# philip-bl/dctn

Measured on AMD Instinct MI355X. Metric: EPS-contraction windows/sec (fwd+bwd), higher is better.
Workload: dtype bf16; 1 GPU; cfg2 EPS[(3,4)]+linear bf16 B1024/GPU; parallelism=dp1

## Files before the change

dctn_amd/csrc/eps_mfma.hip:

```cpp
#include "common.h"

#include <cstdlib>
#include <type_traits>

typedef __attribute__((ext_vector_type(8))) __bf16 bf16x8;
typedef __attribute__((ext_vector_type(16))) float f32x16;
typedef __attribute__((ext_vector_type(8))) float f32x8;
typedef __attribute__((ext_vector_type(2))) int int2v;
typedef __attribute__((ext_vector_type(4))) int int4v;
typedef __attribute__((ext_vector_type(2))) float f32x2;

namespace {

constexpr int ilog2(int v) { return v <= 1 ? 0 : 1 + ilog2(v >> 1); }

template <typename S> __device__ __forceinline__ float to_f32(S v) { return (float)v; }

__device__ __forceinline__ float half_sum(float v) {
  const int iv = __float_as_int(v);
  const int2v r = __builtin_amdgcn_permlane32_swap(iv, iv, false, false);
  return __int_as_float(r[0]) + __int_as_float(r[1]);
}

__device__ __forceinline__ void swap_halves(float& a, float& b) {
// ... 38 lines not shown
  return t;
}
__device__ __forceinline__ bf16x8 tr_frag(const short* tile, int ks, const TrLane& t) {
  typedef __attribute__((address_space(3))) s16x4 lds_s16x4;
  const s16x4 lo = __builtin_amdgcn_ds_read_tr16_b64_v4i16((lds_s16x4*)(tile + t.rd_lo + ks * 16 * LROW));
  const s16x4 hi = __builtin_amdgcn_ds_read_tr16_b64_v4i16((lds_s16x4*)(tile + t.rd_hi + ks * 16 * LROW));
  const s16x8 v = {lo[0], lo[1], lo[2], lo[3], hi[0], hi[1], hi[2], hi[3]};
  return __builtin_bit_cast(bf16x8, v);
}

struct FastDiv {
  unsigned M, s1, s2;
};
__device__ __forceinline__ unsigned fdiv(unsigned n, const FastDiv& d) {
  const unsigned t = __umulhi(d.M, n);
  return (t + ((n - t) >> d.s1)) >> d.s2;
}

#define MFMA_MAXN 16
struct MfmaP {
  int C, B, K, O, Ho, Wo;
  int P;
  int npg;
  int spc, nchunks;
  unsigned foffb[MFMA_MAXN];
  unsigned rowoffb[MFMA_MAXN];
  unsigned s1b, s2b, s3b, s4b;
  unsigned x_bytes;
  unsigned o_bytes, o_s1b;
  FastDiv div_wo;
  int rowvec_ok;
  int vec_ok;
  int Cout;
  unsigned hw_rowb, hw_bytes;
  int ncb;
  int skew;
  int opts;
#ifdef DCTN_STAMPS
  unsigned long long* stamps;
#endif
};

#ifdef DCTN_STAMPS
#define DCTN_STAMP(P, SLOT)                                                                      \
  do {                                                                                           \
    __builtin_amdgcn_sched_barrier(0);                                                           \
    unsigned long long t_;                                                                       \
    asm volatile("s_memrealtime %0\n\ts_waitcnt lgkmcnt(0)" : "=s"(t_)::"memory");               \
    if ((P).stamps && threadIdx.x == 0) (P).stamps[(long long)blockIdx.x * 8 + (SLOT)] = t_;     \
    __builtin_amdgcn_sched_barrier(0);                                                           \
  } while (0)
static unsigned long long* g_stamps = nullptr;
void dctn_stamps_set(unsigned long long* p) { g_stamps = p; }
__device__ unsigned long long* g_dev_stamps = nullptr;
void dctn_reduce_stamps_set(unsigned long long* p) { (void)hipMemcpyToSymbol(HIP_SYMBOL(g_dev_stamps), &p, sizeof(p)); }
#define DCTN_STAMP_T(P, SLOT, TID)                                                              \
  do {                                                                                           \
    __builtin_amdgcn_sched_barrier(0);                                                           \
    unsigned long long t_;                                                                       \
    asm volatile("s_memrealtime %0\n\ts_waitcnt lgkmcnt(0)" : "=s"(t_)::"memory");               \
    if ((P).stamps && threadIdx.x == (TID)) (P).stamps[(long long)blockIdx.x * 8 + (SLOT)] = t_;  \
    __builtin_amdgcn_sched_barrier(0);                                                           \
  } while (0)
#define DCTN_STAMP_ROLE_ROW 1024
#define DCTN_STAMP_R(P, SLOT)                                                                    \
  do {                                                                                           \
    __builtin_amdgcn_sched_barrier(0);                                                           \
    unsigned long long t_;                                                                       \
    asm volatile("s_memrealtime %0\n\ts_waitcnt lgkmcnt(0)" : "=s"(t_)::"memory");               \
    if ((P).stamps && threadIdx.x == 64 * 8)                                                     \
      (P).stamps[(long long)(DCTN_STAMP_ROLE_ROW + blockIdx.x) * 8 + (SLOT)] = t_;               \
    __builtin_amdgcn_sched_barrier(0);                                                           \
  } while (0)
#define DCTN_STAMP_WAVE_ROW 1536
#define DCTN_STAMP_W(P, WV)                                                                      \
  do {                                                                                           \
    __builtin_amdgcn_sched_barrier(0);                                                           \
    unsigned long long t_;                                                                       \
    asm volatile("s_memrealtime %0\n\ts_waitcnt lgkmcnt(0)" : "=s"(t_)::"memory");               \
    if ((P).stamps && (threadIdx.x & 63) == 0 && (WV) < 8)                                        \
      (P).stamps[(long long)(DCTN_STAMP_WAVE_ROW + blockIdx.x) * 8 + (WV)] = t_;                 \
    __builtin_amdgcn_sched_barrier(0);                                                           \
  } while (0)
#define DCTN_STAMP_G(SLOT)                                                                       \
  do {                                                                                           \
    __builtin_amdgcn_sched_barrier(0);                                                           \
    unsigned long long t_;                                                                       \
    asm volatile("s_memrealtime %0\n\ts_waitcnt lgkmcnt(0)" : "=s"(t_)::"memory");               \
    if (g_dev_stamps && threadIdx.x == 0) g_dev_stamps[(long long)blockIdx.x * 8 + (SLOT)] = t_;  \
    __builtin_amdgcn_sched_barrier(0);                                                           \
  } while (0)
#else
#define DCTN_STAMP(P, SLOT) do { } while (0)
#define DCTN_STAMP_T(P, SLOT, TID) do { } while (0)
#define DCTN_STAMP_G(SLOT) do { } while (0)
#define DCTN_STAMP_R(P, SLOT) do { } while (0)
#define DCTN_STAMP_W(P, WV) do { } while (0)
#endif

typedef __attribute__((ext_vector_type(4))) unsigned u32x4;
typedef __attribute__((ext_vector_type(2))) unsigned u32x2;
typedef __attribute__((ext_vector_type(2))) __bf16 bf16x2;

__device__ __forceinline__ __amdgpu_buffer_rsrc_t make_rsrc(const void* ptr, unsigned bytes) {
  return __builtin_amdgcn_make_buffer_rsrc(const_cast<void*>(ptr), 0, (int)bytes, 0x00020000);
}

template <typename S, int N, bool VEC, int ROWS>
struct RawWindow {
  u32x4 row[ROWS > 0 ? ROWS : 1];
  unsigned v[(ROWS == 0 && VEC) ? N * (int)(sizeof(S) / 2) : 1];
  unsigned e[(ROWS == 0 && !VEC) ? 2 * N : 1];
};

template <typename S, int N, bool VEC, int ROWS>
__device__ __forceinline__ void issue_window(__amdgpu_buffer_rsrc_t rs, unsigned voff, unsigned soff,
                                             const MfmaP& p, RawWindow<S, N, VEC, ROWS>& raw) {
  if constexpr (ROWS > 0) {
#pragma unroll
    for (int rw = 0; rw < ROWS; ++rw)
      raw.row[rw] = __builtin_amdgcn_raw_buffer_load_b128(rs, voff, soff + p.rowoffb[rw], 0);
  } else if constexpr (VEC) {
#pragma unroll
    for (int n = 0; n < N; ++n) {
      if constexpr (sizeof(S) == 2) {
        raw.v[n] = __builtin_amdgcn_raw_buffer_load_b32(rs, voff, soff + p.foffb[n], 0);
      } else {
        const u32x2 t = __builtin_amdgcn_raw_buffer_load_b64(rs, voff, soff + p.foffb[n], 0);
        raw.v[2 * n] = t.x;
        raw.v[2 * n + 1] = t.y;
      }
    }
  } else {
#pragma unroll
    for (int n = 0; n < N; ++n)
#pragma unroll
      for (int q = 0; q < 2; ++q) {
        if constexpr (sizeof(S) == 2)
          raw.e[2 * n + q] = (unsigned)(unsigned short)__builtin_amdgcn_raw_buffer_load_b16(
              rs, voff, soff + p.foffb[n] + q * p.s4b, 0);
        else
          raw.e[2 * n + q] = __builtin_amdgcn_raw_buffer_load_b32(rs, voff, soff + p.foffb[n] + q * p.s4b, 0);
      }
  }
}

template <typename S, int N, bool VEC, int ROWS>
__device__ __forceinline__ void unpack_window(const RawWindow<S, N, VEC, ROWS>& raw, float (&xv)[N][2]) {
  if constexpr (ROWS > 0) {
    constexpr int KK = N / ROWS;
    constexpr int CC = ROWS * ROWS / N;
#pragma unroll
    for (int rw = 0; rw < ROWS; ++rw) {
      const unsigned d[4] = {raw.row[rw].x, raw.row[rw].y, raw.row[rw].z, raw.row[rw].w};
#pragma unroll
      for (int dw = 0; dw < KK; ++dw) {
        const int n = ((rw / CC) * KK + dw) * CC + (rw % CC);
        xv[n][0] = __uint_as_float(d[dw] << 16);
        xv[n][1] = __uint_as_float(d[dw] & 0xffff0000u);
      }
    }
  } else if constexpr (VEC) {
#pragma unroll
    for (int n = 0; n < N; ++n) {
      if constexpr (sizeof(S) == 2) {
        xv[n][0] = __uint_as_float(raw.v[n] << 16);
        xv[n][1] = __uint_as_float(raw.v[n] & 0xffff0000u);
      } else {
        xv[n][0] = __uint_as_float(raw.v[2 * n]);
        xv[n][1] = __uint_as_float(raw.v[2 * n + 1]);
      }
    }
  } else {
#pragma unroll
    for (int n = 0; n < N; ++n)
#pragma unroll
      for (int q = 0; q < 2; ++q)
        xv[n][q] = sizeof(S) == 2 ? __uint_as_float(raw.e[2 * n + q] << 16) : __uint_as_float(raw.e[2 * n + q]);
  }
}
// ... 403 lines not shown
        for (int bh = 0; bh < BN / 2; ++bh) {
          const f32x2 mm = bmul2(ph[bh], f32x2{xv[N - 1][0], xv[N - 1][1]});
          m0[bh] = mm[0];
          m1[bh] = mm[1];
          swap_halves(m0[bh], m1[bh]);
        }
      }
      float res0[OP], res1[OP];
#pragma unroll
      for (int o = 0; o < OP; ++o) { res0[o] = 0.f; res1[o] = 0.f; }
#pragma unroll
      for (int t = 0; t < MT; ++t) {
#pragma unroll
        for (int set = 0; set < 2; ++set) {
          f32x16 acc;
#pragma unroll
          for (int v = 0; v < 16; ++v) acc[v] = 0.f;
#pragma unroll
          for (int s = 0; s < KS; ++s)
            acc = __builtin_amdgcn_mfma_f32_32x32x16_bf16(cf[t][s], set ? pf1[s] : pf0[s], acc, 0, 0, 0);
#pragma unroll
          for (int v = 0; v < 16; v += 2) {
            const int code = (t << 4) | ((v >> 2) << 2) | (v & 3);
            const float mm = set ? m1[code >> LOGO] : m0[code >> LOGO];
            float* dst = set ? res1 : res0;
            const int o = code & (OP - 1);
            const f32x2 r = bfma2(mm, f32x2{acc[v], acc[v + 1]}, f32x2{dst[o], dst[o + 1]});
            dst[o] = r[0];
            dst[o + 1] = r[1];
          }
        }
      }
      unsigned pk[OP / 2];
#pragma unroll
      for (int i = 0; i < OP / 2; ++i) {
        float a0 = res0[2 * i], a1 = res1[2 * i], c0 = res0[2 * i + 1], c1 = res1[2 * i + 1];
        swap_halves(a0, a1);
        swap_halves(c0, c1);
        pk[i] = pack_bf16(a0 + a1, c0 + c1);
      }
      if constexpr (OP == 2) {
        __builtin_amdgcn_raw_buffer_store_b32(pk[0], rs_o, voff_o, (unsigned)b * p.o_s1b, 0);
        *reinterpret_cast<unsigned*>(tile + (b - g0) * SROW + lane * OP) = pk[0];
      } else if constexpr (OP == 4) {
        __builtin_amdgcn_raw_buffer_store_b64(u32x2{pk[0], pk[1]}, rs_o, voff_o, (unsigned)b * p.o_s1b, 0);
        *reinterpret_cast<u32x2*>(tile + (b - g0) * SROW + lane * OP) = u32x2{pk[0], pk[1]};
      } else {
#pragma unroll
        for (int i = 0; i < OP / 8; ++i) {
          const u32x4 q = u32x4{pk[4 * i], pk[4 * i + 1], pk[4 * i + 2], pk[4 * i + 3]};
          __builtin_amdgcn_raw_buffer_store_b128(q, rs_o, voff_o, (unsigned)b * p.o_s1b + 16u * i, 0);
          *reinterpret_cast<u32x4*>(tile + (b - g0) * SROW + lane * OP + 8 * i) = q;
        }
      }
      if (b == b0) DCTN_STAMP(p, 2);
    }
    wave_lds_sync();
    f32x4v hd = {0.f, 0.f, 0.f, 0.f};
#pragma unroll
    for (int ks = 0; ks < HK; ++ks) {
      const bf16x8 fb = *reinterpret_cast<const bf16x8*>(brd + 32 * ks);
      hd = __builtin_amdgcn_mfma_f32_16x16x32_bf16(wf[ks], fb, hd, 0, 0, 0);
    }
    wave_lds_sync();
    {
      const int sl = lane & 15, cb = 4 * (lane >> 4);
      if (sl < g1 - g0) {
#pragma unroll
        for (int v = 0; v < 4; ++v) hsum[grp & 1][sl][cb + v][wv] = hd[v];
      }
    }
    DCTN_STAMP(p, 3);
    __syncthreads();
    for (int e = tid; e < (g1 - g0) * p.Cout; e += (int)blockDim.x) {
      const int sl = e / p.Cout, c = e - sl * p.Cout;
      float t = (float)bias[c];
      for (int w = 0; w < nwv; ++w) t += hsum[grp & 1][sl][c][w];
      logits[(long long)(g0 + sl) * p.Cout + c] = (bf16_t)t;
    }
  }
  DCTN_STAMP(p, 4);
}

constexpr int HEADT_WAVES = 16;
constexpr int HEADT_GS = 4;
constexpr int HEADT_MAXKS = 6;
constexpr int headt_pitch(int F) { return (F + 31) / 32 * 32 + 8; }

template <int N0, int N1, int OP, int ROWS, bool BLK4>
__global__ __launch_bounds__(64 * HEADT_WAVES) void eps_fwd_head_q2reg_t_k(const bf16_t* __restrict__ x,
                                                                           const bf16_t* __restrict__ core,
                                                                           const bf16_t* __restrict__ hw,
                                                                           const bf16_t* __restrict__ bias,
                                                                           bf16_t* __restrict__ out,
                                                                           bf16_t* __restrict__ logits, MfmaP p) {
  typedef bf16_t S;
  typedef __attribute__((ext_vector_type(4))) float f32x4v;
  constexpr int N = N0 + N1, A = 1 << N0, BN = 1 << N1, KS = A / 16, MT = BN * OP / 32;
  constexpr int LOGO = ilog2(OP);
  constexpr int TOT = A * BN * OP;
  static_assert(OP % 2 == 0 && TOT % 4 == 0, "outputs are handled as bf16 pairs");
  __shared__ __attribute__((aligned(16))) bf16_t cs[TOT];
  __shared__ float hsum[HEADT_WAVES][HEADT_GS][16];
  __shared__ unsigned step_ctr;
  extern __shared__ __attribute__((aligned(16))) short ftile[];
  const int tid = threadIdx.x, lane = tid & 63;
  const int wv = __builtin_amdgcn_readfirstlane(tid >> 6);
  const int b0 = (int)blockIdx.x * p.spc, b1 = b0 + p.spc < p.B ? b0 + p.spc : p.B;
  const int F = p.P * OP, LP = headt_pitch(F);
  const __amdgpu_buffer_rsrc_t rs_x = make_rsrc(x, p.x_bytes), rs_o = make_rsrc(out, p.o_bytes);
  __shared__ float bias_s[16];
  DCTN_STAMP(p, 0);
  float bias_v = 0.f;
  for (int e0 = 0; e0 < TOT; e0 += 4 * 64 * HEADT_WAVES) {
    S tmp[4];
#pragma unroll
    for (int i = 0; i < 4; ++i) {
      const int ec = e0 + tid + i * 64 * HEADT_WAVES, e = ec < TOT ? ec : TOT - 1, o = e % OP, ab = e / OP;
      tmp[i] = core[(long long)ab * p.O + (o < p.O ? o : 0)];
    }
    if (e0 == 0 && wv == 0) bias_v = (float)bias[(lane & 15) < p.Cout ? (lane & 15) : 0];
#pragma unroll
    for (int i = 0; i < 4; ++i) {
      const int e = e0 + tid + i * 64 * HEADT_WAVES, o = e % OP, ab = e / OP, bb = ab % BN, aa = ab / BN;
      const int code = ((bb >> 1) << LOGO) | o;
      const int row = (((code >> 2) & 3) << 3) | ((bb & 1) << 2) | (code & 3);
      const int dst = ((((code >> 4) * KS + (aa >> 4)) * 64 + ((aa >> 3) & 1) * 32 + row) << 3) | (aa & 7);
      if (e < TOT) cs[dst] = o < p.O ? tmp[i] : (bf16_t)0.f;
    }
  }
  if (wv == 0) bias_s[lane & 15] = bias_v;
  for (int e = tid; e < HEADT_GS * (LP - F); e += 64 * HEADT_WAVES) ftile[(e / (LP - F)) * LP + F + e % (LP - F)] = 0;
  __syncthreads();
  bf16x8 cf[MT][KS];
#pragma unroll
  for (int t = 0; t < MT; ++t)
#pragma unroll
    for (int s = 0; s < KS; ++s)
      cf[t][s] = *reinterpret_cast<const bf16x8*>(&cs[((t * KS + s) * 64 + lane) * 8]);
  DCTN_STAMP(p, 1);

  auto lane_at = [&](int pg, bool live, unsigned& voff_x, unsigned& voff_o, int& pos) {
    pos = pg * 64 + lane;
    const bool valid = live && pos < p.P;
    const unsigned pu = (unsigned)(pos < p.P ? pos : p.P - 1);
    const unsigned ho = fdiv(pu, p.div_wo), wo = pu - ho * (unsigned)p.Wo;
    voff_x = valid ? ho * p.s2b + wo * p.s3b : p.x_bytes;
    voff_o = valid ? pu * (unsigned)(OP * 2) : p.o_bytes;
  };
  auto draw = [&]() {
    unsigned v = 0;
    if (lane == 0) v = __hip_atomic_fetch_add(&step_ctr, 1u, __ATOMIC_RELAXED, __HIP_MEMORY_SCOPE_WORKGROUP);
    return (int)__builtin_amdgcn_readfirstlane(v);
  };

  for (int g0 = b0; g0 < b1; g0 += HEADT_GS) {
    const int ng = g0 + HEADT_GS < b1 ? HEADT_GS : b1 - g0;
    const int nsteps = ng * p.npg;
    if (tid == 0) step_ctr = 2 * HEADT_WAVES;
    __syncthreads();
    int cur = wv, nxt = wv + HEADT_WAVES;
    int s = cur / p.npg, pg = cur - s * p.npg, pos;
    unsigned voff_x, voff_o;
    lane_at(pg, cur < nsteps, voff_x, voff_o, pos);
    RawWindow<S, N, true, ROWS> raw;
    issue_window<S, N, true, ROWS>(rs_x, voff_x, (unsigned)(g0 + (cur < nsteps ? s : 0)) * p.s1b, p, raw);
#ifdef DCTN_STAMPS
    bool first_step = true;
#endif
    while (cur < nsteps) {
      float xv[N][2];
      unpack_window<S, N, true, ROWS>(raw, xv);
      const unsigned vo = voff_o, so = (unsigned)(g0 + s) * p.o_s1b;
      short* trow = ftile + s * LP + (pos < p.P ? pos : 0) * OP;
      const bool tvalid = pos < p.P;
      {
        cur = nxt;
        s = cur / p.npg;
        pg = cur - s * p.npg;
        lane_at(pg, cur < nsteps, voff_x, voff_o, pos);
        issue_window<S, N, true, ROWS>(rs_x, voff_x, (unsigned)(g0 + (cur < nsteps ? s : 0)) * p.s1b, p, raw);
        nxt = draw();
        __builtin_amdgcn_sched_barrier(0);
      }
      bf16x8 pf0[KS], pf1[KS];
      build_p0<N0>(xv, pf0, pf1);
#pragma unroll
      for (int s2 = 0; s2 < KS; ++s2) swap_halves(pf0[s2], pf1[s2]);
      float m0[BN / 2], m1[BN / 2];
      {
        float ph[BN / 2];
        ph[0] = xv[N - 2][0];
        ph[1] = xv[N - 2][1];
#pragma unroll
        for (int u = 2; u < N1; ++u)
#pragma unroll
          for (int bh = (1 << (u - 1)) - 1; bh >= 0; --bh) {
            const f32x2 pr = bmul2(ph[bh], f32x2{xv[N - 1 - u][0], xv[N - 1 - u][1]});
            ph[bh] = pr[0];
            ph[bh | (1 << (u - 1))] = pr[1];
          }
#pragma unroll
        for (int bh = 0; bh < BN / 2; ++bh) {
          const f32x2 mm = bmul2(ph[bh], f32x2{xv[N - 1][0], xv[N - 1][1]});
          m0[bh] = mm[0];
          m1[bh] = mm[1];
          swap_halves(m0[bh], m1[bh]);
        }
      }
      float res0[OP], res1[OP];
#pragma unroll
      for (int o = 0; o < OP; ++o) { res0[o] = 0.f; res1[o] = 0.f; }
#pragma unroll
      for (int t = 0; t < MT; ++t) {
#pragma unroll
        for (int set = 0; set < 2; ++set) {
          f32x16 acc;
#pragma unroll
          for (int v = 0; v < 16; ++v) acc[v] = 0.f;
#pragma unroll
          for (int s2 = 0; s2 < KS; ++s2)
            acc = __builtin_amdgcn_mfma_f32_32x32x16_bf16(cf[t][s2], set ? pf1[s2] : pf0[s2], acc, 0, 0, 0);
#pragma unroll
          for (int v = 0; v < 16; v += 2) {
            const int code = (t << 4) | ((v >> 2) << 2) | (v & 3);
            const float mm = set ? m1[code >> LOGO] : m0[code >> LOGO];
            float* dst = set ? res1 : res0;
            const int o = code & (OP - 1);
            const f32x2 r = __builtin_elementwise_fma(f32x2{mm, mm}, f32x2{acc[v], acc[v + 1]}, f32x2{dst[o], dst[o + 1]});
            dst[o] = r[0];
            dst[o + 1] = r[1];
          }
        }
      }
      unsigned pk[OP / 2];
#pragma unroll
      for (int i = 0; i < OP / 2; ++i) {
        float a0 = res0[2 * i], a1 = res1[2 * i], c0 = res0[2 * i + 1], c1 = res1[2 * i + 1];
        swap_halves(a0, a1);
        swap_halves(c0, c1);
        pk[i] = pack_bf16(a0 + a1, c0 + c1);
      }
      if constexpr (OP == 2) {
        if constexpr (!BLK4) __builtin_amdgcn_raw_buffer_store_b32(pk[0], rs_o, vo, so, 0);
        if (tvalid) *reinterpret_cast<unsigned*>(trow) = pk[0];
      } else if constexpr (OP == 4) {
        if constexpr (!BLK4) __builtin_amdgcn_raw_buffer_store_b64(u32x2{pk[0], pk[1]}, rs_o, vo, so, 0);
        if (tvalid) *reinterpret_cast<u32x2*>(trow) = u32x2{pk[0], pk[1]};
      } else {
#pragma unroll
        for (int i = 0; i < OP / 8; ++i) {
          const u32x4 q = u32x4{pk[4 * i], pk[4 * i + 1], pk[4 * i + 2], pk[4 * i + 3]};
          if constexpr (!BLK4) __builtin_amdgcn_raw_buffer_store_b128(q, rs_o, vo, so + 16u * i, 0);
          if (tvalid) *reinterpret_cast<u32x4*>(trow + 8 * i) = q;
        }
      }
#ifdef DCTN_STAMPS
      if (first_step) DCTN_STAMP(p, 2);
      first_step = false;
#endif
    }
    DCTN_STAMP(p, 3);
    DCTN_STAMP_T(p, 4, 64 * (HEADT_WAVES - 1));
    const int nks = (F + 31) / 32;
    const int c = lane & 15, kg = lane >> 4;
    const __amdgpu_buffer_rsrc_t rs_hw = make_rsrc(hw, p.hw_bytes);
    u32x4 wf[HEADT_MAXKS];
#pragma unroll
    for (int i = 0; i < HEADT_MAXKS; ++i) {
      const int ks = wv + HEADT_WAVES * i, k = 32 * ks + 8 * kg;
      const unsigned vo2 = (ks < nks && c < p.Cout && k + 7 < F) ? (unsigned)c * p.hw_rowb + (unsigned)k * 2u : p.hw_bytes;
      wf[i] = __builtin_amdgcn_raw_buffer_load_b128(rs_hw, vo2, 0, 0);
    }
    __syncthreads();
    DCTN_STAMP(p, 5);
    if constexpr (BLK4) {
      static_assert(HEADT_GS == 4, "a group is one block of the blocked4 layout");
      const unsigned sob = (unsigned)(g0 >> 2) * (unsigned)F * 8u;
      for (int f = 2 * tid; f < F; f += 2 * 64 * HEADT_WAVES) {
        unsigned r[HEADT_GS];
#pragma unroll
        for (int i = 0; i < HEADT_GS; ++i) r[i] = i < ng ? *reinterpret_cast<const unsigned*>(ftile + i * LP + f) : 0u;
        const u32x4 q = u32x4{__builtin_amdgcn_perm(r[1], r[0], 0x05040100u), __builtin_amdgcn_perm(r[3], r[2], 0x05040100u),
                              __builtin_amdgcn_perm(r[1], r[0], 0x07060302u), __builtin_amdgcn_perm(r[3], r[2], 0x07060302u)};
        __builtin_amdgcn_raw_buffer_store_b128(q, rs_o, (unsigned)f * 8u, sob, 0);
      }
    }
    __builtin_amdgcn_sched_barrier(0);
    f32x4v hd = {0.f, 0.f, 0.f, 0.f};
    const short* brd = ftile + (c < HEADT_GS ? c : HEADT_GS - 1) * LP + 8 * kg;
#pragma unroll
    for (int i = 0; i < HEADT_MAXKS; ++i) {
      const int ks = wv + HEADT_WAVES * i;
      if (ks < nks) {
        const bf16x8 fb = *reinterpret_cast<const bf16x8*>(brd + 32 * ks);
        hd = __builtin_amdgcn_mfma_f32_16x16x32_bf16(__builtin_bit_cast(bf16x8, wf[i]), fb, hd, 0, 0, 0);
      }
    }
    if (c < HEADT_GS) {
#pragma unroll
      for (int v = 0; v < 4; ++v) hsum[wv][c][4 * kg + v] = hd[v];
    }
    __syncthreads();
    if (tid < HEADT_GS * 16) {
      const int sl = tid >> 4, cc = tid & 15;
      if (sl < ng && cc < p.Cout) {
        float t = bias_s[cc];
#pragma unroll
        for (int w = 0; w < HEADT_WAVES; ++w) t += hsum[w][sl][cc];
        logits[(long long)(g0 + sl) * p.Cout + cc] = (bf16_t)t;
      }
    }
  }
  DCTN_STAMP(p, 6);
}

constexpr int BWD_WAVES = 8;
constexpr size_t dcore_dyn_lds_bytes(int mt) { return (size_t)BWD_WAVES * (1 + mt) * 64 * 32 * sizeof(short); }

__device__ __forceinline__ void head_dw_role_waves(const bf16_t* __restrict__ feat, const bf16_t* __restrict__ dL,
                                                   bf16_t* __restrict__ dW, int B, int Cout, long long F, int n_dw,
                                                   int rw, float* __restrict__ lds, const MfmaP& p);
template <typename S, int N0, int N1, int OP, bool XVEC, bool OVEC, int ROWS, int HEADC, int DWROLE = 0>
__global__ __launch_bounds__(64 * (BWD_WAVES + DWROLE)) void eps_bwd_dcore_q2reg_k(const S* __restrict__ x,
                                                             const S* __restrict__ dY,
                                                             const S* __restrict__ hw,
                                                             const S* __restrict__ feat,
                                                             float* __restrict__ partial,
                                                             float* __restrict__ dwpart, MfmaP p,
                                                             S* __restrict__ dW, int n_dw) {
  constexpr int N = N0 + N1, A = 1 << N0, BN = 1 << N1, KS = A / 16, MT = BN * OP / 32;
  constexpr int AT = A >= 32 ? A / 32 : 1;
  constexpr int LOGO = ilog2(OP);
  constexpr bool LDST = A == 32 && MT <= 2;
  __shared__ float red[BWD_WAVES][32 * 32];
  extern __shared__ __attribute__((aligned(16))) unsigned char dsm[];
  const int tid = threadIdx.x, lane = tid & 63, r = lane & 31, h = lane >> 5, wv = tid >> 6;
  DCTN_STAMP(p, 0);
  if constexpr (DWROLE > 0) {
    static_assert(HEADC > 0 && HEADC <= 16 && LDST && OVEC && XVEC && sizeof(S) == 2 && OP == 4, "the dW role rides the HEADMM path");
    const int rw = __builtin_amdgcn_readfirstlane(wv) - BWD_WAVES;
    if (rw >= 0) {
      head_dw_role_waves(feat, dY, dW, p.B, p.Cout, (long long)p.P * OP, n_dw, rw,
                         reinterpret_cast<float*>(dsm + dcore_dyn_lds_bytes(MT) + 8192), p);
      return;
    }
#ifdef DCTN_DWROLE_PRIO
    __builtin_amdgcn_s_setprio(DCTN_DWROLE_PRIO);
#endif
  }
  short* tiles = reinterpret_cast<short*>(dsm) + wv * ((1 + MT) * 64 * LROW);
  const TrLane trl = tr_lane(lane);

  bf16x8 ident[2];
#pragma unroll
  for (int sp = 0; sp < 2; ++sp)
#pragma unroll
    for (int j = 0; j < 8; ++j) ident[sp][j] = (bf16_t)((16 * sp + 8 * h + j == r) ? 1.f : 0.f);

  f32x16 acc[MT][AT];
#pragma unroll
  for (int t = 0; t < MT; ++t)
#pragma unroll
    for (int a = 0; a < AT; ++a)
#pragma unroll
      for (int v = 0; v < 16; ++v) acc[t][a][v] = 0.f;

  const WaveJob job = wave_job(p, BWD_WAVES, (int)sizeof(S), HEADC > 0);
  const __amdgpu_buffer_rsrc_t rs_x = make_rsrc(x, p.x_bytes);
  const __amdgpu_buffer_rsrc_t rs_dy = make_rsrc(HEADC > 0 ? feat : dY, p.o_bytes);
  constexpr bool HEADMM = HEADC > 0 && HEADC <= 16 && LDST && OVEC && XVEC && sizeof(S) == 2 && OP == 4;
  float hwf[HEADC > 0 && !HEADMM ? HEADC : 1][OP];
  float dwacc[HEADC > 0 && !HEADMM ? HEADC : 1][OP];
#pragma unroll
  for (int c = 0; c < (HEADC > 0 && !HEADMM ? HEADC : 1); ++c)
#pragma unroll
    for (int o = 0; o < OP; ++o) dwacc[c][o] = 0.f;
  constexpr int DLW = HEADC > 0 ? HEADC / 2 : 1;
  const unsigned* dl32 = reinterpret_cast<const unsigned*>(dY);
  unsigned dlraw[DLW];
  RawRow<S, OP> rr[HEADC > 0 && !HEADMM ? HEADC : 1];
  constexpr bool LATE = HEADC > 0 && LDST && !HEADMM;
  auto issue_head_weight = [&]() {
    if constexpr (HEADC > 0 && !HEADMM) {
// ... 933 lines not shown
  constexpr int MT = BN * OP / 32;
  const bool headmm = A == 32 && MT <= 2 && OP == 4 && m.vec_ok;
  if (headmm && (long long)m.B * m.P * OP * 2 >= (1LL << 31)) return DCTN_ERR_UNSUPPORTED;
  const bool gemm = headmm;
  m.skew = headmm ? DCTN_DCORE_SKEW(m.spc) : 0;
  if (m.skew >= m.spc) m.skew = m.spc - 1;

  const dim3 g(grid), b(64 * BWD_WAVES);
  constexpr int NN = N0 + N1;
  constexpr int RW = NN == 9 ? 3 : 4;
  const int n_slices = (int)(((long long)m.P * OP + DWG_BFW - 1) / DWG_BFW);
  bool dwrole = false;
  if constexpr (A == 32 && MT <= 2 && OP == 4) {
    constexpr size_t RDYN = DYN + 8192 + DWR_LDS_BYTES;
#define DCTN_HEAD_ROLE_LAUNCH(ROWSV, HC)                                                                          \
  do {                                                                                                            \
    const void* kfn = (const void*)eps_bwd_dcore_q2reg_k<S, N0, N1, OP, true, true, ROWSV, HC, DWR_WAVES>;        \
    if (dctn_lds_optin(kfn, RDYN)) {                                                                              \
      hipLaunchKernelGGL((eps_bwd_dcore_q2reg_k<S, N0, N1, OP, true, true, ROWSV, HC, DWR_WAVES>), g,             \
                         dim3(64 * (BWD_WAVES + DWR_WAVES)), RDYN, st, (const S*)x, (const S*)dL, (const S*)hw,   \
                         (const S*)feat, (float*)ws, dwpart, m, (S*)dW, dW ? n_slices : 0);                       \
      dwrole = true;                                                                                              \
    }                                                                                                             \
  } while (0)
    if (blk && headmm) {
      if (m.rowvec_ok) {
        if (m.Cout <= 10) DCTN_HEAD_ROLE_LAUNCH(RW, 10); else DCTN_HEAD_ROLE_LAUNCH(RW, 16);
      } else {
        if (m.Cout <= 10) DCTN_HEAD_ROLE_LAUNCH(0, 10); else DCTN_HEAD_ROLE_LAUNCH(0, 16);
      }
    }
#undef DCTN_HEAD_ROLE_LAUNCH
  }
#define DCTN_HEAD_LAUNCH(XV, ROWSV, HC)                                                                        \
  DCTN_DCORE_LAUNCH((eps_bwd_dcore_q2reg_k<S, N0, N1, OP, XV, true, ROWSV, HC>), g, b, (DYN > 0 ? DYN + 8192 : 0), st, (const S*)x, \
                     (const S*)dL, (const S*)hw, (const S*)feat, (float*)ws, dwpart, m, (S*)nullptr, 0)
  if (dwrole) {
  } else if (m.rowvec_ok && m.vec_ok) {
    if (m.Cout <= 10) DCTN_HEAD_LAUNCH(true, RW, 10); else DCTN_HEAD_LAUNCH(true, RW, 16);
  } else if (m.vec_ok) {
    if (m.Cout <= 10) DCTN_HEAD_LAUNCH(true, 0, 10); else DCTN_HEAD_LAUNCH(true, 0, 16);
  } else {
    if (m.Cout <= 10) DCTN_HEAD_LAUNCH(false, 0, 10); else DCTN_HEAD_LAUNCH(false, 0, 16);
  }
#undef DCTN_HEAD_LAUNCH
  DCTN_CHECK_LAUNCH();
  if (m.opts & DCTN_OPT_MAIN_KERNEL_ONLY) return DCTN_PARTIAL;
  const int fw = blk ? DWG_BFW : DWG_FW;
  const int n_core = BN * OP * AT;
  if (dwrole) {
    hipLaunchKernelGGL(eps_head_reduce_k, dim3(n_core + 1), dim3(1024), 0, st, (const float*)ws, (S*)dCore, grid, A, BN, m.O, OP,
                       AT * 32, n_core, (const float*)dwpart, (S*)nullptr, m.ncb, nW, 0, (const S*)dL, (S*)dBias, m.B, m.Cout,
                       (const S*)feat, 0);
    DCTN_CHECK_LAUNCH();
    dctn_set_last_kernel("eps_head_bwd_mfma_q2reg");
    return DCTN_OK;
  }
  const int n_dw = gemm ? (int)(((long long)m.P * OP + fw - 1) / fw) : (int)((nW + 255) / 256);
  const size_t gemm_lds = (size_t)DWG_WAVES * (fw / 4) * 64 * sizeof(float);
  static_assert(DWG_WAVES * 64 == 1024, "the gemm role is the whole workgroup of eps_head_reduce_k");
  if (gemm && !dctn_lds_optin((const void*)eps_head_reduce_k, gemm_lds)) return DCTN_ERR_LAUNCH;
  hipLaunchKernelGGL(eps_head_reduce_k, dim3(n_core + n_dw + 1), dim3(1024), gemm ? gemm_lds : 0, st, (const float*)ws, (S*)dCore,
                     grid, A, BN, m.O, OP, AT * 32, n_core, (const float*)dwpart, (S*)dW, m.ncb, nW, n_dw,
                     (const S*)dL, (S*)dBias, m.B, m.Cout, (const S*)feat, gemm ? (blk ? 2 : 1) : 0);
  DCTN_CHECK_LAUNCH();
  dctn_set_last_kernel("eps_head_bwd_mfma_q2reg");
  return DCTN_OK;
}

template <int N0, int N1, int OP>
int fwd_head_launch_t(const void* x, const void* core, const void* hw, const void* bias, void* out, void* logits,
                      const MfmaP& m_in, hipStream_t st) {
  typedef bf16_t S;
  MfmaP m = m_in;
  const bool blk = (m.opts & DCTN_OPT_HEAD_FEATURES_BLOCKED4) != 0;
  if (m.O != OP || !(m.rowvec_ok && m.vec_ok) || m.npg > HEAD_FWD_MAXPG) return DCTN_ERR_UNSUPPORTED;
  if (((uintptr_t)hw % 16) != 0 || m.hw_rowb % 16 != 0 || ((uintptr_t)out % (blk ? 16 : OP * 2)) != 0) return DCTN_ERR_UNSUPPORTED;
  int nwg = m.B < dctn_dev().cus ? m.B : dctn_dev().cus;
  m.spc = (m.B + nwg - 1) / nwg;
  if (blk) m.spc = (m.spc + HEADT_GS - 1) / HEADT_GS * HEADT_GS;
  nwg = (m.B + m.spc - 1) / m.spc;
  constexpr int RW = (N0 + N1) == 9 ? 3 : 4;
  const long long F = (long long)m.P * OP;
  const bool tk = !(m.opts & DCTN_OPT_SMALL_CHUNKS) && F % 8 == 0 && F <= (long long)HEADT_WAVES * HEADT_MAXKS * 32;
  if (blk) {
    if (!tk || !head_blocked4_ok<N0, N1, OP>(m)) return DCTN_ERR_UNSUPPORTED;
    m.o_bytes = blocked4_bytes(m);
  }
  if (tk) {
    const size_t dyn = (size_t)HEADT_GS * headt_pitch((int)F) * sizeof(short);
#define DCTN_HEADT_LAUNCH(BLK)                                                                                          \
    if (!dctn_lds_optin((const void*)eps_fwd_head_q2reg_t_k<N0, N1, OP, RW, BLK>, dyn)) return DCTN_ERR_UNSUPPORTED;    \
    hipLaunchKernelGGL((eps_fwd_head_q2reg_t_k<N0, N1, OP, RW, BLK>), dim3((unsigned)nwg), dim3(64 * HEADT_WAVES), dyn, st, \
                       (const S*)x, (const S*)core, (const S*)hw, (const S*)bias, (S*)out, (S*)logits, m)
    if (blk) { DCTN_HEADT_LAUNCH(true); } else { DCTN_HEADT_LAUNCH(false); }
#undef DCTN_HEADT_LAUNCH
    DCTN_CHECK_LAUNCH();
    dctn_set_last_kernel("eps_head_fwd_mfma_q2reg");
    return DCTN_OK;
  }
  const dim3 g((unsigned)nwg), b((unsigned)(64 * m.npg));
  hipLaunchKernelGGL((eps_fwd_head_q2reg_k<N0, N1, OP, RW>), g, b, 0, st, (const S*)x, (const S*)core, (const S*)hw,
                     (const S*)bias, (S*)out, (S*)logits, m);
  DCTN_CHECK_LAUNCH();
  dctn_set_last_kernel("eps_head_fwd_mfma_q2reg");
  return DCTN_OK;
}

#define DISPATCH_OP(FN, S, N0, N1, OPV, ...)                         \
  switch (OPV) {                                                     \
    case 2: return FN<S, N0, N1, 2>(__VA_ARGS__);                    \
    case 4: return FN<S, N0, N1, 4>(__VA_ARGS__);                    \
    case 8: return FN<S, N0, N1, 8>(__VA_ARGS__);                    \
    case 16: return FN<S, N0, N1, 16>(__VA_ARGS__);                  \
  }                                                                  \
  return DCTN_ERR_UNSUPPORTED;

template <typename S>
int fwd_dispatch(const void* x, const void* core, void* out, double* stats, const MfmaP& m, int N, int op,
                 hipStream_t st) {
  if (N == 9) { DISPATCH_OP(fwd_launch_t, S, 5, 4, op, x, core, out, stats, m, st) }
  DISPATCH_OP(fwd_launch_t, S, 4, 4, op, x, core, out, stats, m, st)
}

template <typename S>
int bwd_dispatch(const void* x, const void* dY, void* dCore, void* ws, const MfmaP& m, int N,
                 int op, hipStream_t st) {
  if (N == 9) { DISPATCH_OP(bwd_launch_t, S, 5, 4, op, x, dY, dCore, ws, m, st) }
  DISPATCH_OP(bwd_launch_t, S, 4, 4, op, x, dY, dCore, ws, m, st)
}

}

int eps_fwd_mfma(const void* x, const void* core, void* out, const EpsP& p, int dtype,
                 int precision, hipStream_t st, double* stats) {
  if (!family_ok(p, dtype, precision)) return DCTN_ERR_UNSUPPORTED;
  if (!out && !stats) return DCTN_ERR_NULL;
  MfmaP m;
  fill_mp(m, p, x, dtype);
  const int op = next_pow2(p.O) < 2 ? 2 : next_pow2(p.O);
  if (dtype == DCTN_BF16) return fwd_dispatch<bf16_t>(x, core, out, stats, m, p.N, op, st);
  return fwd_dispatch<float>(x, core, out, stats, m, p.N, op, st);
}

size_t eps_bwd_mfma_workspace(const EpsP& p, int dtype, int precision, int need_dx,
                              int need_dcore) {
  (void)need_dx;
  if (!need_dcore || !family_ok(p, dtype, precision)) return 0;
  const int op = next_pow2(p.O) < 2 ? 2 : next_pow2(p.O);
  const int n0 = (p.N + 1) / 2, n1 = p.N - n0;
  const long long A = 1LL << n0, BN = 1LL << n1, acols = A >= 32 ? A : 32;
  return (size_t)dctn_dev().cus * (size_t)(BN * op) * (size_t)acols * sizeof(float);
}

int eps_bwd_mfma(const void* x, const void* core, const void* dY, void* dX, void* dCore, void* ws,
                 size_t ws_bytes, const EpsP& p, int dtype, int precision, hipStream_t st) {
  (void)core;
  if (dX || !dCore) return DCTN_ERR_UNSUPPORTED;
  if (!family_ok(p, dtype, precision)) return DCTN_ERR_UNSUPPORTED;
  if (!ws || ws_bytes < eps_bwd_mfma_workspace(p, dtype, precision, 0, 1)) return DCTN_ERR_WORKSPACE;
  MfmaP m;
  fill_mp(m, p, x, dtype);
  const int op = next_pow2(p.O) < 2 ? 2 : next_pow2(p.O);
  if (dtype == DCTN_BF16) return bwd_dispatch<bf16_t>(x, dY, dCore, ws, m, p.N, op, st);
  return bwd_dispatch<float>(x, dY, dCore, ws, m, p.N, op, st);
}

// ... 56 lines not shown
```

Measured before the change: 28.39 billion windows/s.

## Overlap forward head tail with EPS steps via per-position-group completion counters

```diff
diff --git a/dctn_amd/csrc/eps_mfma.hip b/dctn_amd/csrc/eps_mfma.hip
--- a/dctn_amd/csrc/eps_mfma.hip
+++ b/dctn_amd/csrc/eps_mfma.hip
@@ -144,6 +144,16 @@
       (P).stamps[(long long)(DCTN_STAMP_WAVE_ROW + blockIdx.x) * 8 + (WV)] = t_;                 \
     __builtin_amdgcn_sched_barrier(0);                                                           \
   } while (0)
+#define DCTN_STAMP_FWAVE_ROW 2048
+#define DCTN_STAMP_FW(P, KIND, WV)                                                               \
+  do {                                                                                           \
+    __builtin_amdgcn_sched_barrier(0);                                                           \
+    unsigned long long t_;                                                                       \
+    asm volatile("s_memrealtime %0\n\ts_waitcnt lgkmcnt(0)" : "=s"(t_)::"memory");               \
+    if ((P).stamps && (threadIdx.x & 63) == 0 && blockIdx.x < 256)                               \
+      (P).stamps[(long long)(DCTN_STAMP_FWAVE_ROW + blockIdx.x * 8 + (KIND) * 2 + ((WV) >> 3)) * 8 + ((WV) & 7)] = t_; \
+    __builtin_amdgcn_sched_barrier(0);                                                           \
+  } while (0)
 #define DCTN_STAMP_G(SLOT)                                                                       \
   do {                                                                                           \
     __builtin_amdgcn_sched_barrier(0);                                                           \
@@ -158,6 +168,7 @@
 #define DCTN_STAMP_G(SLOT) do { } while (0)
 #define DCTN_STAMP_R(P, SLOT) do { } while (0)
 #define DCTN_STAMP_W(P, WV) do { } while (0)
+#define DCTN_STAMP_FW(P, KIND, WV) do { } while (0)
 #endif
 
 typedef __attribute__((ext_vector_type(4))) unsigned u32x4;
@@ -727,6 +738,12 @@
   DCTN_STAMP(p, 4);
 }
 
+#ifdef DCTN_FWD_HEAD_SERIAL_TAIL
+constexpr bool HEADT_OVERLAP = false;
+#else
+constexpr bool HEADT_OVERLAP = true;
+#endif
+constexpr int HEADT_MAXPG = 16;
 constexpr int HEADT_WAVES = 16;
 constexpr int HEADT_GS = 4;
 constexpr int HEADT_MAXKS = 6;
@@ -748,6 +765,8 @@
   __shared__ __attribute__((aligned(16))) bf16_t cs[TOT];
   __shared__ float hsum[HEADT_WAVES][HEADT_GS][16];
   __shared__ unsigned step_ctr;
+  __shared__ unsigned tail_ctr;
+  __shared__ unsigned done[HEADT_MAXPG];
   extern __shared__ __attribute__((aligned(16))) short ftile[];
   const int tid = threadIdx.x, lane = tid & 63;
   const int wv = __builtin_amdgcn_readfirstlane(tid >> 6);
@@ -798,14 +817,41 @@
     if (lane == 0) v = __hip_atomic_fetch_add(&step_ctr, 1u, __ATOMIC_RELAXED, __HIP_MEMORY_SCOPE_WORKGROUP);
     return (int)__builtin_amdgcn_readfirstlane(v);
   };
+  auto draw_tail = [&]() {
+    unsigned v = 0;
+    if (lane == 0) v = __hip_atomic_fetch_add(&tail_ctr, 1u, __ATOMIC_RELAXED, __HIP_MEMORY_SCOPE_WORKGROUP);
+    return (int)__builtin_amdgcn_readfirstlane(v);
+  };
 
   for (int g0 = b0; g0 < b1; g0 += HEADT_GS) {
     const int ng = g0 + HEADT_GS < b1 ? HEADT_GS : b1 - g0;
     const int nsteps = ng * p.npg;
+    auto deal = [&](int t, int& s_, int& pg_) {
+      if constexpr (HEADT_OVERLAP) {
+        pg_ = t / ng;
+        s_ = t - pg_ * ng;
+      } else {
+        s_ = t / p.npg;
+        pg_ = t - s_ * p.npg;
+      }
+    };
+    auto wait_pg = [&](int pgw) {
+      for (;;) {
+        const unsigned d = __hip_atomic_load(&done[pgw], __ATOMIC_RELAXED, __HIP_MEMORY_SCOPE_WORKGROUP);
+        if ((int)__builtin_amdgcn_readfirstlane(d) == ng) break;
+        __builtin_amdgcn_s_sleep(1);
+      }
+      asm volatile("s_waitcnt lgkmcnt(0)" ::: "memory");
+    };
     if (tid == 0) step_ctr = 2 * HEADT_WAVES;
+    if constexpr (HEADT_OVERLAP) {
+      if (tid == 0) tail_ctr = 0;
+      if (tid < HEADT_MAXPG) done[tid] = 0;
+    }
     __syncthreads();
     int cur = wv, nxt = wv + HEADT_WAVES;
-    int s = cur / p.npg, pg = cur - s * p.npg, pos;
+    int s, pg, pos;
+    deal(cur, s, pg);
     unsigned voff_x, voff_o;
     lane_at(pg, cur < nsteps, voff_x, voff_o, pos);
     RawWindow<S, N, true, ROWS> raw;
@@ -819,10 +865,10 @@
       const unsigned vo = voff_o, so = (unsigned)(g0 + s) * p.o_s1b;
       short* trow = ftile + s * LP + (pos < p.P ? pos : 0) * OP;
       const bool tvalid = pos < p.P;
+      const int pgc = pg;
       {
         cur = nxt;
-        s = cur / p.npg;
-        pg = cur - s * p.npg;
+        deal(cur, s, pg);
         lane_at(pg, cur < nsteps, voff_x, voff_o, pos);
         issue_window<S, N, true, ROWS>(rs_x, voff_x, (unsigned)(g0 + (cur < nsteps ? s : 0)) * p.s1b, p, raw);
         nxt = draw();
@@ -900,51 +946,117 @@
           if (tvalid) *reinterpret_cast<u32x4*>(trow + 8 * i) = q;
         }
       }
+      if constexpr (HEADT_OVERLAP) {
+        asm volatile("s_waitcnt lgkmcnt(0)" ::: "memory");
+        if (lane == 0) __hip_atomic_fetch_add(&done[pgc], 1u, __ATOMIC_RELAXED, __HIP_MEMORY_SCOPE_WORKGROUP);
+      }
 #ifdef DCTN_STAMPS
-      if (first_step) DCTN_STAMP(p, 2);
+      if (first_step) {
+        DCTN_STAMP(p, 2);
+        DCTN_STAMP_FW(p, 0, wv);
+      }
       first_step = false;
 #endif
     }
     DCTN_STAMP(p, 3);
     DCTN_STAMP_T(p, 4, 64 * (HEADT_WAVES - 1));
+    DCTN_STAMP_FW(p, 1, wv);
     const int nks = (F + 31) / 32;
     const int c = lane & 15, kg = lane >> 4;
     const __amdgpu_buffer_rsrc_t rs_hw = make_rsrc(hw, p.hw_bytes);
-    u32x4 wf[HEADT_MAXKS];
-#pragma unroll
-    for (int i = 0; i < HEADT_MAXKS; ++i) {
-      const int ks = wv + HEADT_WAVES * i, k = 32 * ks + 8 * kg;
-      const unsigned vo2 = (ks < nks && c < p.Cout && k + 7 < F) ? (unsigned)c * p.hw_rowb + (unsigned)k * 2u : p.hw_bytes;
-      wf[i] = __builtin_amdgcn_raw_buffer_load_b128(rs_hw, vo2, 0, 0);
-    }
-    __syncthreads();
-    DCTN_STAMP(p, 5);
-    if constexpr (BLK4) {
-      static_assert(HEADT_GS == 4, "a group is one block of the blocked4 layout");
-      const unsigned sob = (unsigned)(g0 >> 2) * (unsigned)F * 8u;
-      for (int f = 2 * tid; f < F; f += 2 * 64 * HEADT_WAVES) {
-        unsigned r[HEADT_GS];
-#pragma unroll
-        for (int i = 0; i < HEADT_GS; ++i) r[i] = i < ng ? *reinterpret_cast<const unsigned*>(ftile + i * LP + f) : 0u;
-        const u32x4 q = u32x4{__builtin_amdgcn_perm(r[1], r[0], 0x05040100u), __builtin_amdgcn_perm(r[3], r[2], 0x05040100u),
-                              __builtin_amdgcn_perm(r[1], r[0], 0x07060302u), __builtin_amdgcn_perm(r[3], r[2], 0x07060302u)};
-        __builtin_amdgcn_raw_buffer_store_b128(q, rs_o, (unsigned)f * 8u, sob, 0);
-      }
-    }
-    __builtin_amdgcn_sched_barrier(0);
-    f32x4v hd = {0.f, 0.f, 0.f, 0.f};
-    const short* brd = ftile + (c < HEADT_GS ? c : HEADT_GS - 1) * LP + 8 * kg;
-#pragma unroll
-    for (int i = 0; i < HEADT_MAXKS; ++i) {
-      const int ks = wv + HEADT_WAVES * i;
-      if (ks < nks) {
-        const bf16x8 fb = *reinterpret_cast<const bf16x8*>(brd + 32 * ks);
-        hd = __builtin_amdgcn_mfma_f32_16x16x32_bf16(__builtin_bit_cast(bf16x8, wf[i]), fb, hd, 0, 0, 0);
-      }
-    }
-    if (c < HEADT_GS) {
-#pragma unroll
-      for (int v = 0; v < 4; ++v) hsum[wv][c][4 * kg + v] = hd[v];
+    if constexpr (HEADT_OVERLAP) {
+      const int nst = BLK4 ? p.npg : 0;
+#ifdef DCTN_STAMPS
+      bool first_chain = true;
+#endif
+      for (;;) {
+        const int tk = draw_tail();
+        if (tk >= nst + HEADT_WAVES) break;
+        if constexpr (BLK4) {
+          if (tk < nst) {
+            static_assert(HEADT_GS == 4, "a group is one block of the blocked4 layout");
+            const unsigned sob = (unsigned)(g0 >> 2) * (unsigned)F * 8u;
+            const int fa = tk * 64 * OP, fe = fa + 64 * OP < F ? fa + 64 * OP : F;
+            wait_pg(tk);
+            for (int f = fa + 2 * lane; f < fe; f += 2 * 64) {
+              unsigned r[HEADT_GS];
+#pragma unroll
+              for (int i = 0; i < HEADT_GS; ++i) r[i] = i < ng ? *reinterpret_cast<const unsigned*>(ftile + i * LP + f) : 0u;
+              const u32x4 q = u32x4{__builtin_amdgcn_perm(r[1], r[0], 0x05040100u), __builtin_amdgcn_perm(r[3], r[2], 0x05040100u),
+                                    __builtin_amdgcn_perm(r[1], r[0], 0x07060302u), __builtin_amdgcn_perm(r[3], r[2], 0x07060302u)};
+              __builtin_amdgcn_raw_buffer_store_b128(q, rs_o, (unsigned)f * 8u, sob, 0);
+            }
+            if (tk == nst - 1) DCTN_STAMP_T(p, 7, 64 * wv);
+            continue;
+          }
+        }
+        const int v = tk - nst;
+#ifdef DCTN_STAMPS
+        if (first_chain) DCTN_STAMP_FW(p, 2, wv);
+        first_chain = false;
+#endif
+        u32x4 wf[HEADT_MAXKS];
+#pragma unroll
+        for (int i = 0; i < HEADT_MAXKS; ++i) {
+          const int ks = v + HEADT_WAVES * i, k = 32 * ks + 8 * kg;
+          const unsigned vo2 = (ks < nks && c < p.Cout && k + 7 < F) ? (unsigned)c * p.hw_rowb + (unsigned)k * 2u : p.hw_bytes;
+          wf[i] = __builtin_amdgcn_raw_buffer_load_b128(rs_hw, vo2, 0, 0);
+        }
+        f32x4v hd = {0.f, 0.f, 0.f, 0.f};
+        const short* brd = ftile + (c < HEADT_GS ? c : HEADT_GS - 1) * LP + 8 * kg;
+#pragma unroll
+        for (int i = 0; i < HEADT_MAXKS; ++i) {
+          const int ks = v + HEADT_WAVES * i;
+          if (ks < nks) {
+            wait_pg(ks / (2 * OP));
+            const bf16x8 fb = *reinterpret_cast<const bf16x8*>(brd + 32 * ks);
+            hd = __builtin_amdgcn_mfma_f32_16x16x32_bf16(__builtin_bit_cast(bf16x8, wf[i]), fb, hd, 0, 0, 0);
+          }
+        }
+        if (c < HEADT_GS) {
+#pragma unroll
+          for (int u = 0; u < 4; ++u) hsum[v][c][4 * kg + u] = hd[u];
+        }
+        DCTN_STAMP_FW(p, 3, wv);
+      }
+      DCTN_STAMP(p, 5);
+    } else {
+      u32x4 wf[HEADT_MAXKS];
+#pragma unroll
+      for (int i = 0; i < HEADT_MAXKS; ++i) {
+        const int ks = wv + HEADT_WAVES * i, k = 32 * ks + 8 * kg;
+        const unsigned vo2 = (ks < nks && c < p.Cout && k + 7 < F) ? (unsigned)c * p.hw_rowb + (unsigned)k * 2u : p.hw_bytes;
+        wf[i] = __builtin_amdgcn_raw_buffer_load_b128(rs_hw, vo2, 0, 0);
+      }
+      __syncthreads();
+      DCTN_STAMP(p, 5);
+      if constexpr (BLK4) {
+        static_assert(HEADT_GS == 4, "a group is one block of the blocked4 layout");
+        const unsigned sob = (unsigned)(g0 >> 2) * (unsigned)F * 8u;
+        for (int f = 2 * tid; f < F; f += 2 * 64 * HEADT_WAVES) {
+          unsigned r[HEADT_GS];
+#pragma unroll
+          for (int i = 0; i < HEADT_GS; ++i) r[i] = i < ng ? *reinterpret_cast<const unsigned*>(ftile + i * LP + f) : 0u;
+          const u32x4 q = u32x4{__builtin_amdgcn_perm(r[1], r[0], 0x05040100u), __builtin_amdgcn_perm(r[3], r[2], 0x05040100u),
+                                __builtin_amdgcn_perm(r[1], r[0], 0x07060302u), __builtin_amdgcn_perm(r[3], r[2], 0x07060302u)};
+          __builtin_amdgcn_raw_buffer_store_b128(q, rs_o, (unsigned)f * 8u, sob, 0);
+        }
+      }
+      __builtin_amdgcn_sched_barrier(0);
+      f32x4v hd = {0.f, 0.f, 0.f, 0.f};
+      const short* brd = ftile + (c < HEADT_GS ? c : HEADT_GS - 1) * LP + 8 * kg;
+#pragma unroll
+      for (int i = 0; i < HEADT_MAXKS; ++i) {
+        const int ks = wv + HEADT_WAVES * i;
+        if (ks < nks) {
+          const bf16x8 fb = *reinterpret_cast<const bf16x8*>(brd + 32 * ks);
+          hd = __builtin_amdgcn_mfma_f32_16x16x32_bf16(__builtin_bit_cast(bf16x8, wf[i]), fb, hd, 0, 0, 0);
+        }
+      }
+      if (c < HEADT_GS) {
+#pragma unroll
+        for (int v = 0; v < 4; ++v) hsum[wv][c][4 * kg + v] = hd[v];
+      }
     }
     __syncthreads();
     if (tid < HEADT_GS * 16) {
@@ -2044,7 +2156,8 @@
   nwg = (m.B + m.spc - 1) / m.spc;
   constexpr int RW = (N0 + N1) == 9 ? 3 : 4;
   const long long F = (long long)m.P * OP;
-  const bool tk = !(m.opts & DCTN_OPT_SMALL_CHUNKS) && F % 8 == 0 && F <= (long long)HEADT_WAVES * HEADT_MAXKS * 32;
+  const bool tk = !(m.opts & DCTN_OPT_SMALL_CHUNKS) && F % 8 == 0 && F <= (long long)HEADT_WAVES * HEADT_MAXKS * 32 &&
+                  m.npg <= HEADT_MAXPG;
   if (blk) {
     if (!tk || !head_blocked4_ok<N0, N1, OP>(m)) return DCTN_ERR_UNSUPPORTED;
     m.o_bytes = blocked4_bytes(m);
```

Result: slower. 27.63 billion windows/s (-2.7%).
